# LDEO-CREW/Pythonic-DISORT

Measured on AMD Instinct MI355X. Metric: column-solves/sec (32 streams, 20 layers), higher is better.
Workload: dtype f64

## Files before the change

### pythonic-disort_amd/csrc/rtd_eig.hip

```cpp
#include <cstdlib>
#include <type_traits>

#include "rtd_device.h"

namespace {

#define RTD_FENCE() asm volatile("" ::: "memory")
#ifndef RTD_XOR_DPP
#define RTD_XOR_DPP 0x818E
#endif

constexpr __host__ __device__ int dpp_xor_ctrl(int mask) {
  return mask == 1 ? 0xB1 : mask == 2 ? 0x4E : mask == 3 ? 0x1B : mask == 7 ? 0x141 : mask == 8 ? 0x128 : mask == 15 ? 0x140 : -1;
}

template <int MASK>
__device__ __forceinline__ double xor_lane(double v) {
  if constexpr (MASK >= 32) return __shfl_xor(v, MASK, 64);
  int lo = __double2loint(v), hi = __double2hiint(v);
  constexpr int ctrl = dpp_xor_ctrl(MASK);
  if constexpr (ctrl >= 0 && ((RTD_XOR_DPP >> MASK) & 1)) {
    lo = __builtin_amdgcn_update_dpp(0, lo, ctrl, 0xF, 0xF, true);
    hi = __builtin_amdgcn_update_dpp(0, hi, ctrl, 0xF, 0xF, true);
  } else {
// ... 102 lines not shown
template <int B, int E, typename F>
__device__ __forceinline__ void static_for(F&& f) {
  if constexpr (B < E) {
    f(std::integral_constant<int, B>{});
    static_for<B + 1, E>(f);
  }
}

template <int NP, int K>
__device__ __forceinline__ double bcast_lane(double v) {
  if constexpr (NP == 16) {
    int lo = __double2loint(v), hi = __double2hiint(v);
    lo = __builtin_amdgcn_update_dpp(0, lo, 0x150 + K, 0xF, 0xF, true);
    hi = __builtin_amdgcn_update_dpp(0, hi, 0x150 + K, 0xF, 0xF, true);
    return __hiloint2double(hi, lo);
  } else if constexpr (NP == 64) {
    return __hiloint2double(__builtin_amdgcn_readlane(__double2hiint(v), K), __builtin_amdgcn_readlane(__double2loint(v), K));
  } else {
    return __shfl(v, K, NP);
  }
}

template <int NP, int K, int I, bool ORDERED = false>
struct CholRowDpp {
  static __device__ __forceinline__ void run(double (&col)[NP], const double f) {
    if constexpr (ORDERED) {
      if constexpr (I == K + 1 || I == NP - 1)
        asm volatile("v_fmac_f64_dpp %0, -%0, %1 row_newbcast:%2 row_mask:0xf bank_mask:0xf\n\ts_nop 1" : "+v"(col[I]) : "v"(f), "n"(K % 16));
      else
        asm volatile("v_fmac_f64_dpp %0, -%0, %1 row_newbcast:%2 row_mask:0xf bank_mask:0xf" : "+v"(col[I]) : "v"(f), "n"(K % 16));
    } else {
      if constexpr (I == K + 1 || I == NP - 1)
        asm("v_fmac_f64_dpp %0, -%0, %1 row_newbcast:%2 row_mask:0xf bank_mask:0xf\n\ts_nop 1" : "+v"(col[I]) : "v"(f), "n"(K % 16));
      else
        asm("v_fmac_f64_dpp %0, -%0, %1 row_newbcast:%2 row_mask:0xf bank_mask:0xf" : "+v"(col[I]) : "v"(f), "n"(K % 16));
    }
    CholRowDpp<NP, K, I + 1, ORDERED>::run(col, f);
  }
};
template <int NP, int K, bool ORDERED>
struct CholRowDpp<NP, K, NP, ORDERED> {
  static __device__ __forceinline__ void run(double (&)[NP], const double) {}
};

template <int NP, int K>
struct CholStep {
  static __device__ __forceinline__ void run(double (&col)[NP], double& diag, const int j) {
    const double akk = bcast_lane<NP, K>(col[K]);
    const double f = (j > K) ? col[K] * fast_rcp(akk) : 0.0;
    diag = (j == K) ? akk : diag;
    if constexpr (RTD_CHOL_FMAC_DPP && NP == 16) {
      CholRowDpp<NP, K, K + 1>::run(col, f);
    } else {
#pragma unroll
      for (int i = K + 1; i < NP; ++i) col[i] = fma(-bcast_lane<NP, K>(col[i]), f, col[i]);
    }
    CholStep<NP, K + 1>::run(col, diag, j);
  }
};
template <int NP>
struct CholStep<NP, NP> {
  static __device__ __forceinline__ void run(double (&)[NP], double&, const int) {}
};
template <int I>
struct RowFmacDpp {
  static __device__ __forceinline__ void run(double (&acc)[32], const double y0, const double y1, const double coef) {
    asm("v_fmac_f64_dpp %0, %1, %2 row_newbcast:%3 row_mask:0xf bank_mask:0xf" : "+v"(acc[I]) : "v"(y0), "v"(coef), "n"(I));
    asm("v_fmac_f64_dpp %0, %1, %2 row_newbcast:%3 row_mask:0xf bank_mask:0xf" : "+v"(acc[16 + I]) : "v"(y1), "v"(coef), "n"(I));
    if constexpr (I + 1 < 16) RowFmacDpp<I + 1>::run(acc, y0, y1, coef);
  }
};

template <int I>
struct RowFmacDpp64 {
  static __device__ __forceinline__ void run(double (&acc)[64], const double (&y)[4], const double coef) {
    asm("v_fmac_f64_dpp %0, %1, %2 row_newbcast:%3 row_mask:0xf bank_mask:0xf" : "+v"(acc[I]) : "v"(y[0]), "v"(coef), "n"(I));
    asm("v_fmac_f64_dpp %0, %1, %2 row_newbcast:%3 row_mask:0xf bank_mask:0xf" : "+v"(acc[16 + I]) : "v"(y[1]), "v"(coef), "n"(I));
    asm("v_fmac_f64_dpp %0, %1, %2 row_newbcast:%3 row_mask:0xf bank_mask:0xf" : "+v"(acc[32 + I]) : "v"(y[2]), "v"(coef), "n"(I));
    asm("v_fmac_f64_dpp %0, %1, %2 row_newbcast:%3 row_mask:0xf bank_mask:0xf" : "+v"(acc[48 + I]) : "v"(y[3]), "v"(coef), "n"(I));
    if constexpr (I + 1 < 16) RowFmacDpp64<I + 1>::run(acc, y, coef);
  }
};

template <int K>
__device__ __forceinline__ void fmac_bcast(double& acc, const double src, const double mul) {
  asm("v_fmac_f64_dpp %0, %1, %2 row_newbcast:%3 row_mask:0xf bank_mask:0xf" : "+v"(acc) : "v"(src), "v"(mul), "n"(K));
}

template <int NP>
struct LRowN {
  double g[NP / 16];
  template <int R, bool PACKED>
  static __device__ __forceinline__ LRowN load(const double* L_, const int t) {
    constexpr int off = PACKED ? R * (R + 1) / 2 : R * (NP + 1);
    LRowN x;
#pragma unroll
    for (int gi = 0; gi < NP / 16; ++gi) x.g[gi] = 16 * gi <= R ? L_[off + 16 * gi + t] : 0.0;
    return x;
  }
};
template <int NP, int I, int IEND>
struct AxpyRowN {
  static __device__ __forceinline__ void run(double (&acc)[NP], const LRowN<NP>& row, const double mul) {
    if constexpr (I < IEND) {
      fmac_bcast<I % 16>(acc[I], row.g[I / 16], mul);
      AxpyRowN<NP, I + 1, IEND>::run(acc, row, mul);
    }
  }
};
template <int NP, int I, int IEND>
struct DotRowN {
  static __device__ __forceinline__ void run(double (&a)[NP / 16], const LRowN<NP>& row, const double (&v)[NP]) {
    if constexpr (I < IEND) {
      fmac_bcast<I % 16>(a[I / 16], row.g[I / 16], v[I]);
      DotRowN<NP, I + 1, IEND>::run(a, row, v);
    }
  }
};

template <int NP>
__device__ __forceinline__ double transpose_reduce_scaled(const double (&a)[NP], const double s, const int j) {
  constexpr int O = NP / 2;
  const bool hi = (j & O) != 0;
  double v[O];
#pragma unroll
  for (int i = 0; i < O; ++i) v[i] = level_add<O, true>(a[i] * s, a[i + O] * s, hi);
  return transpose_reduce<O>(v, j);
}
template <int NP>
__device__ __forceinline__ double transpose_reduce_scaled2(const double (&a)[NP], const double s, const double (&b)[NP], const double t, const int j) {
  constexpr int O = NP / 2;
  const bool hi = (j & O) != 0;
  double v[O];
#pragma unroll
  for (int i = 0; i < O; ++i) v[i] = level_add<O, true>(fma(b[i], t, a[i] * s), fma(b[i + O], t, a[i + O] * s), hi);
  return transpose_reduce<O>(v, j);
}

template <int K>
__device__ __forceinline__ double row_bcast16(double v) {
  int lo = __double2loint(v), hi = __double2hiint(v);
  lo = __builtin_amdgcn_update_dpp(0, lo, 0x150 + K, 0xF, 0xF, true);
  hi = __builtin_amdgcn_update_dpp(0, hi, 0x150 + K, 0xF, 0xF, true);
  return __hiloint2double(hi, lo);
}
template <int K, int KEND>
struct CholPanel32 {
  static __device__ __forceinline__ void run(double (&col)[32], double& diag, double& dmine, const int row, const int jj) {
    constexpr int PR = K / 16, KL = K % 16;
    const double akk = row_bcast16<KL>(col[K]);
    const double r = fast_rcp(akk);
    const bool mine = row == PR;
    const double f = (mine && jj > KL) ? col[K] * r : 0.0;
    diag = (mine && jj == KL) ? akk : diag;
    dmine = (mine && jj == KL) ? r : dmine;
    CholRowDpp<32, K, K + 1, true>::run(col, f);
    if constexpr (K + 1 < KEND) CholPanel32<K + 1, KEND>::run(col, diag, dmine, row, jj);
  }
};
__device__ __forceinline__ double cholesky_columns32(double (&col)[32], const int j, double* scratch) {
  typedef double v4d __attribute__((ext_vector_type(4)));
  const int lane = threadIdx.x, g = lane >> 5, row = (lane >> 4) & 1, jj = lane & 15;
  double diag = 1.0, dmine = 0.0;
  CholPanel32<0, 16>::run(col, diag, dmine, row, jj);
  double* sX = scratch;
  double* sXd = scratch + 512;
  __syncthreads();
  if (row == 0) {
#pragma unroll
    for (int i = 0; i < 16; ++i) {
      sX[(g * 16 + jj) * 16 + i] = col[16 + i];
      sXd[(g * 16 + jj) * 16 + i] = col[16 + i] * dmine;
    }
  }
  __syncthreads();
  v4d acc[2];
#pragma unroll
  for (int pg = 0; pg < 2; ++pg) {
    acc[pg] = v4d{0.0, 0.0, 0.0, 0.0};
#pragma unroll
    for (int t = 0; t < 4; ++t) {
      const int e = (pg * 16 + 4 * t + (lane >> 4)) * 16 + (lane & 15);
      acc[pg] = __builtin_amdgcn_mfma_f64_16x16x4f64(sXd[e], sX[e], acc[pg], 0, 0, 0);
    }
  }
  __syncthreads();
  double* sS = scratch;
#pragma unroll
  for (int pg = 0; pg < 2; ++pg)
#pragma unroll
    for (int q = 0; q < 4; ++q) sS[(pg * 16 + 4 * q + (lane >> 4)) * 16 + (lane & 15)] = acc[pg][q];
  __syncthreads();
  if (row == 1) {
#pragma unroll
    for (int i = 0; i < 16; ++i) col[16 + i] -= sS[(g * 16 + i) * 16 + jj];
  }
  CholPanel32<16, 32>::run(col, diag, dmine, row, jj);
  const double rinv = fast_rsqrt(diag);
#pragma unroll
  for (int i = 0; i < 32; ++i) col[i] = (i >= j) ? col[i] * rinv : 0.0;
  __syncthreads();
  return rinv;
}

template <int NP>
__device__ __forceinline__ double cholesky_columns(double (&col)[NP], const int j) {
  double diag = 1.0;
  CholStep<NP, 0>::run(col, diag, j);
  const double rinv = fast_rsqrt(diag);
#pragma unroll
  for (int i = 0; i < NP; ++i) col[i] = (i >= j) ? col[i] * rinv : 0.0;
  return rinv;
}

struct ProbId {
  long pid;
  int c, m, l;
  int mg;
  bool valid;
// ... 140 lines not shown
    const double delta = ay - ax;
    const double g2 = 2.0 * gamma;
    const float df = (float)delta, gf = (float)g2;
    const float r2f = fmaf(df, df, fmaf(gf, gf, 1e-36f));
    const float rhof = r2f * __builtin_amdgcn_rsqf(r2f);
    const float denf = df + copysignf(rhof, df);
    const double tt = (double)(gf * __builtin_amdgcn_rcpf(denf));
    const double t2 = fma(tt, tt, 1.0);
    const double c = fast_rsqrt(t2);
    const double cinv = t2 * c;
    notconv |= (gamma * gamma > RTD_JAC_TOL * ax * ay) ? 1 : 0;
    const double nax = fma(-tt, gamma, ax), nay = fma(tt, gamma, ay);
    const double a = -tt * (sy * rx), b = tt * (sx * ry);
    const double nsx = c * sx, nsy = c * sy, nrx = cinv * rx, nry = cinv * ry;
    if constexpr (SW == 0) {
#pragma unroll
      for (int i = 0; i < H; ++i) {
        const double xi = xh[i], yi = yh[i];
        xh[i] = fma(a, yi, xi);
        yh[i] = xor_lane<MK>(fma(b, xi, yi));
      }
      ax = nax;
      ay = xor_lane<MK>(nay);
      sx = nsx;
      rx = nrx;
      sy = xor_lane<MK>(nsy);
      ry = xor_lane<MK>(nry);
    } else {
      const bool swp = (p & SW) != 0;
      const double pxx = swp ? b : 1.0, pxy = swp ? 1.0 : a, pyx = swp ? 1.0 : b, pyy = swp ? a : 1.0;
#pragma unroll
      for (int i = 0; i < H; ++i) {
        const double xi = xh[i], yi = yh[i];
        xh[i] = fma(pxy, yi, pxx * xi);
        yh[i] = xor_lane<MK>(fma(pyy, yi, pyx * xi));
      }
      ax = swp ? nay : nax;
      ay = xor_lane<MK>(swp ? nax : nay);
      sx = swp ? nsy : nsx;
      rx = swp ? nry : nrx;
      sy = xor_lane<MK>(swp ? nsx : nsy);
      ry = xor_lane<MK>(swp ? nrx : nry);
      const int t = swp ? iy : ix;
      iy = swp ? ix : iy;
      ix = t;
    }
    iy = xor_lane_i<MK>(iy);
    FastPairStep<NP, S + 1>::run(xh, yh, ax, ay, ix, iy, p, notconv, sx, sy, rx, ry);
  }
};
template <int NP>
struct FastPairStep<NP, NP - 1> {
  static __device__ __forceinline__ void run(double (&)[NP / 2], double (&)[NP / 2], double&, double&, int&, int&, const int, int&,
                                             double&, double&, double&, double&) {}
};

__host__ __device__ constexpr int tri(int r, int c) { return r * (r + 1) / 2 + c; }

#ifdef RTD_EIG_STAMPS
#define RTD_ESTAMP(k)                                      \
  {                                                        \
    __builtin_amdgcn_sched_barrier(0);                     \
    est[k] = (long long)__builtin_amdgcn_s_memtime();      \
    __builtin_amdgcn_sched_barrier(0);                     \
  }
#else
#define RTD_ESTAMP(k)
#endif

template <int NP, int JV>
__global__ __launch_bounds__(64, (NP <= 16 ? RTD_EIGEN_WAVES : NP == 32 ? RTD_EIGEN32_WAVES : 1)) void rtd_eigen_kernel(RtdDev d) {
  constexpr int GPW = 64 / NP;
  constexpr bool PACKED = NP == 32;
  constexpr int LD = NP + 1;
  constexpr int LSIZE = PACKED ? NP * (NP + 1) / 2 : NP * LD;
  __shared__ double sL[GPW][LSIZE];
  auto lix = [](const int r, const int c) { return PACKED ? tri(r, c) : r * LD + c; };
  __shared__ double sV[GPW][4][NP];
  constexpr int TROWS = NP == 32 ? 32 : 1;
  __shared__ double sTab[NP == 32 ? TROWS * NP : 1];
  __shared__ double sCoef[NP == 32 ? GPW * TROWS : 1];
  __shared__ double sY0[NP == 32 ? TROWS : 1];
  double w[NP];
  double xe_sum = 0.0, xo_sum = 0.0;
#ifdef RTD_EIG_STAMPS
  long long est[12];
  for (int k = 0; k < 12; ++k) est[k] = 0;
  int est_sweeps = 0;
#endif
  RTD_ESTAMP(0);
  double mu0_c = 1.0, I0_c = 0.0;
  if (d.beam) {
    const int c0 = locate<NP>(d).c;
    mu0_c = d.mu0[c0];
    I0_c = d.I0[c0];
  }
  {
  const int grp = threadIdx.x / NP, j = threadIdx.x % NP;
  const ProbId id = locate<NP>(d);
  const int P = d.P, m = id.m, c = id.c, l = id.l;
  double* L_ = sL[grp];
  double* dinv = sV[grp][3];
  const double* wl = d.wleg + ((long)c * d.L + l) * P;
  const double om = d.omega[(long)c * d.L + l];
  const double* Ym = d.Y + (long)m * P * NP;

  const double invmu_j = d.invmu[j], S_j = d.S[j];
  if constexpr (JV == 3 && NP == 16) {
    typedef double v4d __attribute__((ext_vector_type(4)));
    typedef unsigned int u2 __attribute__((ext_vector_type(2)));
    const int tx = threadIdx.x, i16 = tx & 15, k4 = tx >> 4;
    int chunk = (int)((long)blockIdx.x % (d.nsel > 0 ? d.nsel : (d.ln + GPW - 1) / GPW));
    if (d.nsel > 0) chunk = d.chunk_sel[(long)c * d.nsel + chunk];
    if (chunk < 0) chunk = (d.ln + GPW - 1) / GPW;
    double cm_ = 0.0;
    for (int ell = id.mg + j; ell < P; ell += NP) cm_ = fmax(cm_, fabs(0.5 * om * wl[ell]));
    const unsigned long long livemask = __ballot(cm_ > 1e-8);
    if (d.beam && ((livemask >> (NP * grp)) & 0xffffull)) {
      const double* Y0b = d.Y0 + ((long)c * d.M + m) * P;
      for (int ell = id.mg; ell < P; ell += 2) {
        xe_sum = fma(om * wl[ell] * Ym[(long)ell * NP + j], Y0b[ell], xe_sum);
        if (ell + 1 < P) xo_sum = fma(om * wl[ell + 1] * Ym[(long)(ell + 1) * NP + j], Y0b[ell + 1], xo_sum);
      }
    }
    const double S_i = d.S[i16], invmu_c = d.invmu[i16];
    v4d accP[GPW], accQ[GPW];
#pragma unroll
    for (int g = 0; g < GPW; ++g)
#pragma unroll
      for (int q = 0; q < 4; ++q) accP[g][q] = accQ[g][q] = (4 * q + k4 == i16) ? invmu_c : 0.0;
    const double* wlg[GPW];
    double omg[GPW];
#pragma unroll
    for (int g = 0; g < GPW; ++g) {
      const int slot = chunk * GPW + g;
      const int sl = slot < d.ln ? slot : d.ln - 1;
      const int lg = d.ln == d.L ? d.lperm[(long)c * d.L + sl] : d.l0 + sl;
      wlg[g] = d.wleg + ((long)c * d.L + lg) * P;
      omg[g] = ((livemask >> (NP * g)) & 0xffffull) ? -d.omega[(long)c * d.L + lg] : 0.0;
    }
    for (int base = id.mg; base < P; base += 8) {
      const int le = base + 2 * k4, lo = le + 1;
      const double ye = le < P ? Ym[(long)le * NP + i16] * S_i : 0.0;
      const double yo = lo < P ? Ym[(long)lo * NP + i16] * S_i : 0.0;
#pragma unroll
      for (int g = 0; g < GPW; ++g) {
        const double ce = le < P ? omg[g] * wlg[g][le] : 0.0, co = lo < P ? omg[g] * wlg[g][lo] : 0.0;
        accP[g] = __builtin_amdgcn_mfma_f64_16x16x4f64(ce * ye, ye, accP[g], 0, 0, 0);
        accQ[g] = __builtin_amdgcn_mfma_f64_16x16x4f64(co * yo, yo, accQ[g], 0, 0, 0);
      }
    }
    double pcol[NP], qcol[NP];
    auto transpose4 = [](const v4d (&acc)[GPW], const int q, double (&out)[NP]) {
      unsigned r[4][2];
#pragma unroll
      for (int g = 0; g < 4; ++g) {
        r[g][0] = (unsigned)__double2loint(acc[g][q]);
        r[g][1] = (unsigned)__double2hiint(acc[g][q]);
      }
#pragma unroll
      for (int h = 0; h < 2; ++h) {
        const u2 s01 = __builtin_amdgcn_permlane16_swap(r[0][h], r[1][h], false, false);
        const u2 s23 = __builtin_amdgcn_permlane16_swap(r[2][h], r[3][h], false, false);
        const u2 t02 = __builtin_amdgcn_permlane32_swap(s01[0], s23[0], false, false);
        const u2 t13 = __builtin_amdgcn_permlane32_swap(s01[1], s23[1], false, false);
        r[0][h] = t02[0];
        r[2][h] = t02[1];
        r[1][h] = t13[0];
        r[3][h] = t13[1];
      }
#pragma unroll
      for (int k = 0; k < 4; ++k) out[4 * q + k] = __hiloint2double((int)r[k][1], (int)r[k][0]);
    };
    if constexpr (GPW == 4) {
#pragma unroll
      for (int q = 0; q < 4; ++q) {
        transpose4(accP, q, pcol);
        transpose4(accQ, q, qcol);
      }
    }
    dinv[j] = cholesky_columns<NP>(pcol, j);
    cholesky_columns<NP>(qcol, j);
#pragma unroll
    for (int i = 0; i < NP; ++i)
        if (!PACKED || j <= i) L_[lix(i, 0) + j] = pcol[i];
    __syncthreads();
#pragma unroll
    for (int i = 0; i < NP; ++i) {
      double a = 0.0;
#pragma unroll
      for (int r = i; r < NP; ++r) a += L_[lix(r, i)] * qcol[r];
      w[i] = a;
    }
  } else if constexpr (NP == 32) {
    const int le = id.mg + 2 * j, lo = le + 1;
    const double wle = le < P ? wl[le] : 0.0, wlo = lo < P ? wl[lo] : 0.0;
    const double* Y0b = d.Y0 + ((long)c * d.M + m) * P;
    const double y0e = (d.beam && le < P) ? Y0b[le] : 0.0, y0o = (d.beam && lo < P) ? Y0b[lo] : 0.0;
    double cmax = fmax(fabs(0.5 * om * wle), fabs(0.5 * om * wlo));
    cmax = fmax(cmax, xor_lane<1>(cmax));
    cmax = fmax(cmax, xor_lane<2>(cmax));
    cmax = fmax(cmax, xor_lane<4>(cmax));
    cmax = fmax(cmax, xor_lane<8>(cmax));
    cmax = fmax(cmax, xor_lane<16>(cmax));
    const double live = (cmax > 1e-8) ? 1.0 : 0.0;
    auto assemble = [&](const int first, const double wmine, const double y0mine, double (&col)[NP], double& beam_sum) {
      const int nrows = (P - first + 1) / 2;
      __syncthreads();
      {
        constexpr int TRIPS = TROWS * (NP / 2) / 64;
        double2 v[TRIPS];
#pragma unroll
        for (int t = 0; t < TRIPS; ++t) {
          const int idx = t * 64 + (int)threadIdx.x, row = idx / (NP / 2), q = idx % (NP / 2);
          const int ell = first + 2 * row < P ? first + 2 * row : P - 1;
          v[t] = *reinterpret_cast<const double2*>(Ym + (long)ell * NP + 2 * q);
        }
#pragma unroll
        for (int t = 0; t < TRIPS; ++t) {
          const int idx = t * 64 + (int)threadIdx.x;
          if (idx < nrows * (NP / 2)) *reinterpret_cast<double2*>(&sTab[idx * 2]) = v[t];
        }
      }
      sCoef[grp * TROWS + j] = om * wmine;
      if (grp == 0) sY0[j] = y0mine;
      __syncthreads();
      double acc[NP];
#pragma unroll
      for (int i = 0; i < NP; ++i) acc[i] = 0.0;
      const int jj = j & 15;
      for (int k = 0; k < nrows; ++k) {
        const double y0 = sTab[k * NP + jj], y1 = sTab[k * NP + 16 + jj];
        const double coef = sCoef[grp * TROWS + k] * (j < 16 ? y0 : y1);
        beam_sum = fma(live * coef, sY0[k], beam_sum);
        RowFmacDpp<0>::run(acc, y0, y1, coef);
      }
#pragma unroll
      for (int i = 0; i < NP; ++i) col[i] = (i == j ? invmu_j : 0.0) - d.S[i] * (live * acc[i]) * S_j;
    };
    {
      double pcol[NP];
      assemble(id.mg, wle, y0e, pcol, xe_sum);
      RTD_ESTAMP(1);
      dinv[j] = cholesky_columns32(pcol, j, sTab);
      RTD_ESTAMP(2);
#pragma unroll
      for (int i = 0; i < NP; ++i)
        if (!PACKED || j <= i) L_[lix(i, 0) + j] = pcol[i];
    }
    double qcol[NP];
    assemble(id.mg + 1, wlo, y0o, qcol, xo_sum);
    RTD_ESTAMP(3);
    cholesky_columns32(qcol, j, sTab);
    RTD_ESTAMP(4);
    __syncthreads();
    {
      const int t16 = j & 15;
#pragma unroll
      for (int i = 0; i < NP; ++i) w[i] = 0.0;
      static_for<0, NP>([&](auto rc) {
        constexpr int r = decltype(rc)::value;
        const LRowN<NP> row = LRowN<NP>::template load<r, PACKED>(L_, t16);
        AxpyRowN<NP, 0, r + 1>::run(w, row, qcol[r]);
        if constexpr ((r & 3) == 3) RTD_FENCE();
      });
    }
  } else if constexpr (NP == 64) {
    typedef const double __attribute__((address_space(4))) kdouble;
    kdouble* wk = (kdouble*)wl;
    kdouble* Y0k = (kdouble*)(d.Y0 + ((long)c * d.M + m) * P);
    const int jj = j & 15;
    const bool jr1 = (j & 16) != 0, jr2 = (j & 32) != 0;
    double cmax = 0.0;
    {
      const int l0 = id.mg + j, l1 = l0 + NP;
      if (l0 < P) cmax = fabs(0.5 * om * wl[l0]);
      if (l1 < P) cmax = fmax(cmax, fabs(0.5 * om * wl[l1]));
      cmax = fmax(cmax, xor_lane<1>(cmax));
      cmax = fmax(cmax, xor_lane<2>(cmax));
      cmax = fmax(cmax, xor_lane<4>(cmax));
      cmax = fmax(cmax, xor_lane<8>(cmax));
      cmax = fmax(cmax, xor_lane<16>(cmax));
      cmax = fmax(cmax, xor_lane<32>(cmax));
    }
    const double live = (cmax > 1e-8) ? 1.0 : 0.0;
    auto assemble = [&](const int first, double (&col)[NP], double& beam_sum) {
      double acc[NP];
#pragma unroll
      for (int i = 0; i < NP; ++i) acc[i] = 0.0;
      constexpr int CH = 8;
      double yv[CH][4], yn[CH][4], wv[CH], wn[CH], y0v[CH], y0n[CH];
#pragma unroll
      for (int e = 0; e < CH; ++e) {
        const int ell = first + 2 * e < P ? first + 2 * e : P - 1;
#pragma unroll
        for (int g = 0; g < 4; ++g) yv[e][g] = Ym[(long)ell * NP + 16 * g + jj];
        wv[e] = wk[ell];
        y0v[e] = Y0k[ell];
      }
#pragma unroll 1
      for (int base = first; base < P; base += 2 * CH) {
#pragma unroll
        for (int e = 0; e < CH; ++e) {
          const int ell = base + 2 * (CH + e) < P ? base + 2 * (CH + e) : P - 1;
#pragma unroll
          for (int g = 0; g < 4; ++g) yn[e][g] = Ym[(long)ell * NP + 16 * g + jj];
          wn[e] = wk[ell];
          y0n[e] = Y0k[ell];
        }
#pragma unroll
        for (int e = 0; e < CH; ++e) {
          if (base + 2 * e < P) {
            const double ylo = jr1 ? yv[e][1] : yv[e][0], yhi = jr1 ? yv[e][3] : yv[e][2];
            const double coef = om * wv[e] * (jr2 ? yhi : ylo);
            beam_sum = fma(coef, y0v[e], beam_sum);
            RowFmacDpp64<0>::run(acc, yv[e], coef);
          }
        }
#pragma unroll
        for (int e = 0; e < CH; ++e) {
#pragma unroll
          for (int g = 0; g < 4; ++g) yv[e][g] = yn[e][g];
          wv[e] = wn[e];
          y0v[e] = y0n[e];
        }
      }
      beam_sum *= live;
#pragma unroll
      for (int i = 0; i < NP; ++i) col[i] = (i == j ? invmu_j : 0.0) - d.S[i] * (live * acc[i]) * S_j;
    };
    {
      double pcol[NP];
      assemble(id.mg, pcol, xe_sum);
      RTD_ESTAMP(1);
      dinv[j] = cholesky_columns<NP>(pcol, j);
      RTD_ESTAMP(2);
#pragma unroll
      for (int i = 0; i < NP; ++i) L_[lix(i, 0) + j] = pcol[i];
    }
    double qcol[NP];
    assemble(id.mg + 1, qcol, xo_sum);
    RTD_ESTAMP(3);
    cholesky_columns<NP>(qcol, j);
    RTD_ESTAMP(4);
    __syncthreads();
    {
      const int t16 = j & 15;
#pragma unroll
      for (int i = 0; i < NP; ++i) w[i] = 0.0;
      static_for<0, NP>([&](auto rc) {
        constexpr int r = decltype(rc)::value;
        const LRowN<NP> row = LRowN<NP>::template load<r, PACKED>(L_, t16);
        AxpyRowN<NP, 0, r + 1>::run(w, row, qcol[r]);
        if constexpr ((r & 3) == 3) RTD_FENCE();
      });
    }
  } else {
  double acc_e[NP], acc_o[NP];
#pragma unroll
  for (int i = 0; i < NP; ++i) acc_e[i] = acc_o[i] = 0.0;
  double cmax = 0.0;
  const double* Y0b = d.Y0 + ((long)c * d.M + m) * P;
  for (int ell = id.mg; ell < P; ell += 2) {
    {
      const double cl = 0.5 * om * wl[ell];
      cmax = fmax(cmax, fabs(cl));
      const double* Yr = Ym + (long)ell * NP;
      const double coef = 2.0 * cl * Yr[j];
      if (d.beam) xe_sum = fma(coef, Y0b[ell], xe_sum);
#pragma unroll
      for (int i = 0; i < NP; ++i) acc_e[i] += coef * Yr[i];
    }
    if (ell + 1 < P) {
      const double cl = 0.5 * om * wl[ell + 1];
      cmax = fmax(cmax, fabs(cl));
      const double* Yr = Ym + (long)(ell + 1) * NP;
      const double coef = 2.0 * cl * Yr[j];
      if (d.beam) xo_sum = fma(coef, Y0b[ell + 1], xo_sum);
#pragma unroll
      for (int i = 0; i < NP; ++i) acc_o[i] += coef * Yr[i];
    }
  }
  if (!(cmax > 1e-8)) {
#pragma unroll
    for (int i = 0; i < NP; ++i) acc_e[i] = acc_o[i] = 0.0;
    xe_sum = xo_sum = 0.0;
  }
  {
    double pcol[NP], qcol[NP];
#pragma unroll
    for (int i = 0; i < NP; ++i) {
      const double Si = d.S[i];
      pcol[i] = (i == j ? invmu_j : 0.0) - Si * acc_e[i] * S_j;
      qcol[i] = (i == j ? invmu_j : 0.0) - Si * acc_o[i] * S_j;
    }
    RTD_ESTAMP(1);
    dinv[j] = cholesky_columns<NP>(pcol, j);
    RTD_ESTAMP(2);
    RTD_ESTAMP(3);
    cholesky_columns<NP>(qcol, j);
    RTD_ESTAMP(4);
#pragma unroll
    for (int i = 0; i < NP; ++i)
        if (!PACKED || j <= i) L_[lix(i, 0) + j] = pcol[i];
    __syncthreads();
#pragma unroll
    for (int i = 0; i < NP; ++i) {
      double a = 0.0;
#pragma unroll
      for (int r = i; r < NP; ++r) a += L_[lix(r, i)] * qcol[r];
      w[i] = a;
    }
  }
  }
  RTD_ESTAMP(5);
  int nsweep = 0;
  bool converged = false;
  {
    constexpr int H = NP / 2;
    const int u = j / H, p = j % H;
    double xh[H], yh[H];
#pragma unroll
    for (int i = 0; i < H; ++i) {
      const double recv = xor_lane<H>(u ? w[i] : w[H + i]);
      xh[i] = u ? recv : w[i];
      yh[i] = u ? w[H + i] : recv;
    }
    int ix = p, iy = p + H;
    for (int sweep = 0; sweep < 40; ++sweep) {
      int notconv = 0;
      double ax = 0.0, ay = 0.0;
#pragma unroll
      for (int i = 0; i < H; ++i) {
        ax = fma(xh[i], xh[i], ax);
        ay = fma(yh[i], yh[i], ay);
      }
      ax += xor_lane<H>(ax);
      ay += xor_lane<H>(ay);
      if constexpr (RTD_JAC_FAST && NP >= 32) {
        double sx = 1.0, sy = 1.0, rx = 1.0, ry = 1.0;
        FastPairStep<NP, 0>::run(xh, yh, ax, ay, ix, iy, p, notconv, sx, sy, rx, ry);
#pragma unroll
        for (int i = 0; i < H; ++i) {
          xh[i] *= sx;
          yh[i] *= sy;
        }
      } else {
        PairStep<NP, 0>::run(xh, yh, ax, ay, ix, iy, p, notconv);
      }
      ++nsweep;
      if (!__any(notconv)) {
        converged = true;
        break;
      }
    }
#pragma unroll
    for (int i = 0; i < H; ++i) {
      const double recv = xor_lane<H>(u ? xh[i] : yh[i]);
      w[i] = u ? recv : xh[i];
      w[H + i] = u ? yh[i] : recv;
    }
    int* where = reinterpret_cast<int*>(sV[grp][0]);
    where[u ? iy : ix] = j;
    __syncthreads();
    const int src = where[j];
#pragma unroll
    for (int i = 0; i < NP; ++i) w[i] = __shfl(w[i], src, NP);
    __syncthreads();
  }
  RTD_ESTAMP(6);
#ifdef RTD_EIG_STAMPS
  est_sweeps = nsweep;
#endif
  if (threadIdx.x == 0 && nsweep > *(volatile int*)d.sweeps) atomicMax(d.sweeps, nsweep);
  if (!converged && threadIdx.x == 0) rtd_raise(d, RTD_ST_JACOBI, id.mg, id.c);
  }
  int tx = threadIdx.x;
  asm volatile("" : "+v"(tx));
  const int grp = tx / NP, j = tx % NP;
  const ProbId id = locate<NP>(d, tx);
  const int P = d.P, m = id.m, c = id.c, l = id.l;
  const bool valid = id.valid;
  const long base = id.pid;
  double* L_ = sL[grp];
  double* v0 = sV[grp][0];
  double* v1 = sV[grp][1];
  double* v2 = sV[grp][2];
  double* dinv = sV[grp][3];
  const double* wl = d.wleg + ((long)c * d.L + l) * P;
  const double om = d.omega[(long)c * d.L + l];
  const double* Ym = d.Y + (long)m * P * NP;
  double invmu_j = d.invmu[j], T_j = d.T[j];
  double dts;
  {
    const double* ts0 = d.taus0 + (long)c * (d.L + 1);
    dts = ts0[l + 1] - ts0[l];
  }
  double k2 = 0.0;
#pragma unroll
  for (int i = 0; i < NP; ++i) k2 += w[i] * w[i];
  const double rk0 = fast_rsqrt(k2), kj = k2 * rk0;
  if (valid && !(k2 > 0.0 && k2 < 1e300)) rtd_raise(d, RTD_ST_CHOL, id.mg, id.c);
  double zc[NP];
  {
#pragma unroll
    for (int i = 0; i < NP; ++i) zc[i] = w[i] * rk0;
  }

  double ya[NP];
  if constexpr (NP >= 32) {
    const int t16 = j & 15;
#pragma unroll
    for (int i = 0; i < NP; ++i) ya[i] = zc[i];
    static_for<0, NP>([&](auto kc) {
      constexpr int r = NP - 1 - decltype(kc)::value;
      ya[r] *= dinv[r];
      if constexpr (r > 0) {
        const LRowN<NP> row = LRowN<NP>::template load<r, PACKED>(L_, t16);
        AxpyRowN<NP, 0, r>::run(ya, row, -ya[r]);
      }
      if constexpr ((r & 3) == 0) RTD_FENCE();
    });
  } else {
#pragma unroll
  for (int i = NP - 1; i >= 0; --i) {
    double a = zc[i];
#pragma unroll
    for (int r = i + 1; r < NP; ++r) a -= L_[lix(r, i)] * ya[r];
    ya[i] = a * dinv[i];
    RTD_FENCE();
  }
  }
  RTD_ESTAMP(7);
  double ekj = 0.0;
  if constexpr (NP == 32) ekj = exp(-kj * dts);
  asm volatile("" : "+v"(invmu_j), "+v"(T_j), "+v"(dts));
  auto store_Y = [&]() {
    if constexpr (NP == 32) {
      asm volatile("" : "+v"(ya[0]), "+v"(ya[1]), "+v"(ya[2]), "+v"(ya[3]), "+v"(ya[4]), "+v"(ya[5]), "+v"(ya[6]), "+v"(ya[7]), "+v"(ya[8]),
                        "+v"(ya[9]), "+v"(ya[10]), "+v"(ya[11]), "+v"(ya[12]), "+v"(ya[13]), "+v"(ya[14]), "+v"(ya[15]));
      asm volatile("" : "+v"(ya[16]), "+v"(ya[17]), "+v"(ya[18]), "+v"(ya[19]), "+v"(ya[20]), "+v"(ya[21]), "+v"(ya[22]), "+v"(ya[23]),
                        "+v"(ya[24]), "+v"(ya[25]), "+v"(ya[26]), "+v"(ya[27]), "+v"(ya[28]), "+v"(ya[29]), "+v"(ya[30]), "+v"(ya[31]));
    }
    if (valid) {
      double* Ym = d.Ym + base * NP * NP;
#pragma unroll
      for (int i = 0; i < NP; ++i) Ym[i * NP + j] = ya[i];
      d.kk[base * NP + j] = kj;
      if constexpr (NP != 32) ekj = exp(-kj * dts);
      d.Ek[base * NP + j] = ekj;
    }
  };
  if constexpr (NP != 32) store_Y();

  double bv_up = 0.0, bv_dn = 0.0;
  if (d.beam) {
    const double mu0 = mu0_c;
    const double fac = I0_c * (0.25 / M_PI) * (id.mg == 0 ? 1.0 : 2.0);
    const double xe = fac * xe_sum, xo = fac * xo_sum;
    const double txd = 2.0 * T_j * xe * invmu_j;
    v0[j] = txd;
    __syncthreads();
    double qv;
    {
      double tq = 0.0;
#pragma unroll
      for (int i = 0; i < NP; ++i) tq += ya[i] * v0[i];
      tq *= k2;
      if constexpr (NP == 32) {
        qv = transpose_reduce_scaled<NP>(ya, tq, j);
      } else {
        double x[NP];
#pragma unroll
        for (int i = 0; i < NP; ++i) x[i] = ya[i] * tq;
        qv = transpose_reduce<NP>(x, j);
      }
    }
    const double rmu0 = fast_rcp(mu0);
    const double rhat = 2.0 * T_j * xo * invmu_j * rmu0 - qv;
    v1[j] = rhat;
    __syncthreads();
    double g = 0.0;
#pragma unroll
    for (int r = 0; r < NP; ++r) g += ((!PACKED || r >= j) ? L_[lix(r, 0) + j] : 0.0) * v1[r];
    v2[j] = g;
    __syncthreads();
    double h = 0.0;
#pragma unroll
    for (int i = 0; i < NP; ++i) h += zc[i] * v2[i];
    h *= fast_rcp(rmu0 * rmu0 - k2);
    double sh, e;
    if constexpr (NP == 32) {
      sh = transpose_reduce_scaled<NP>(ya, h, j);
      e = transpose_reduce_scaled<NP>(zc, h, j);
    } else {
      double x[NP];
#pragma unroll
      for (int i = 0; i < NP; ++i) x[i] = ya[i] * h;
      sh = transpose_reduce<NP>(x, j);
#pragma unroll
      for (int i = 0; i < NP; ++i) x[i] = zc[i] * h;
      e = transpose_reduce<NP>(x, j);
    }
    __syncthreads();
    v2[j] = e;
    __syncthreads();
    double ps = 0.0;
#pragma unroll
    for (int r = 0; r < NP; ++r) ps += ((!PACKED || r <= j) ? L_[lix(j, 0) + r] : 0.0) * v2[r];
    const double rT = fast_rcp(T_j);
    const double s_j = sh * rT;
    const double d_j = mu0 * (txd - ps) * rT;
    bv_up = 0.5 * (s_j + d_j);
    bv_dn = 0.5 * (s_j - d_j);
    if constexpr (NP != 32) {
      if (valid) {
        d.Bv[base * 2 * NP + j] = bv_up;
        d.Bv[base * 2 * NP + NP + j] = bv_dn;
      }
    }
    if (valid && !(fabs(s_j) + fabs(d_j) < 1e300)) rtd_raise(d, RTD_ST_BEAM, id.mg, id.c);
  }
  __syncthreads();
  RTD_ESTAMP(8);
  double aa[NP];
  if constexpr (NP == 32) {
    store_Y();
    const int t16 = j & 15;
    static_for<0, NP>([&](auto rc) {
      constexpr int r = decltype(rc)::value;
      const LRowN<NP> row = LRowN<NP>::template load<r, PACKED>(L_, t16);
      double a[NP / 16] = {};
      DotRowN<NP, 0, r + 1>::run(a, row, zc);
      aa[r] = r >= 16 ? a[0] + a[1] : a[0];
      if constexpr ((r & 3) == 3) RTD_FENCE();
    });
    asm volatile("" : "+v"(aa[0]), "+v"(aa[1]), "+v"(aa[2]), "+v"(aa[3]), "+v"(aa[4]), "+v"(aa[5]), "+v"(aa[6]), "+v"(aa[7]), "+v"(aa[8]),
                      "+v"(aa[9]), "+v"(aa[10]), "+v"(aa[11]), "+v"(aa[12]), "+v"(aa[13]), "+v"(aa[14]), "+v"(aa[15]));
    asm volatile("" : "+v"(aa[16]), "+v"(aa[17]), "+v"(aa[18]), "+v"(aa[19]), "+v"(aa[20]), "+v"(aa[21]), "+v"(aa[22]), "+v"(aa[23]),
                      "+v"(aa[24]), "+v"(aa[25]), "+v"(aa[26]), "+v"(aa[27]), "+v"(aa[28]), "+v"(aa[29]), "+v"(aa[30]), "+v"(aa[31]));
  } else if constexpr (NP == 64) {
    const int t16 = j & 15;
    static_for<0, NP>([&](auto rc) {
      constexpr int r = decltype(rc)::value;
      const LRowN<NP> row = LRowN<NP>::template load<r, PACKED>(L_, t16);
      double a[NP / 16] = {};
      DotRowN<NP, 0, r + 1>::run(a, row, zc);
      aa[r] = (a[0] + a[1]) + (a[2] + a[3]);
      if constexpr ((r & 3) == 3) RTD_FENCE();
    });
  } else {
#pragma unroll
  for (int i = 0; i < NP; ++i) {
    double a = 0.0;
#pragma unroll
    for (int r = 0; r <= i; ++r) a += L_[lix(i, r)] * zc[r];
    aa[i] = a;
    if (NP != 64 || (i & 7) == 7) RTD_FENCE();
  }
  }
  if (valid) {
    double* Am = d.Am + base * NP * NP;
#pragma unroll
    for (int i = 0; i < NP; ++i) Am[i * NP + j] = aa[i];
    if constexpr (NP == 32) {
      if (d.beam) {
        d.Bv[base * 2 * NP + j] = bv_up;
        d.Bv[base * 2 * NP + NP + j] = bv_dn;
      }
    }
  }

  if (d.Ns > 0 && id.mg == 0) {
    const bool act = true;
    double yl[NP == 32 ? NP : 1], al[NP == 32 ? NP : 1];
    if constexpr (NP == 32) {
      const double* Yg = d.Ym + base * NP * NP;
      const double* Ag = d.Am + base * NP * NP;
#pragma unroll
      for (int i = 0; i < NP; ++i) {
        yl[i] = Yg[i * NP + j];
        al[i] = Ag[i * NP + j];
      }
    }
    const auto& ya_t = [&]() -> const double(&)[NP] { if constexpr (NP == 32) return yl; else return ya; }();
    const auto& aa_t = [&]() -> const double(&)[NP] { if constexpr (NP == 32) return al; else return aa; }();
    double zn = 0.0;
#pragma unroll
    for (int i = 0; i < NP; ++i) zn += ya_t[i] * (d.T[i] * d.invmu[i]);
    zn *= -0.5 * kj;
    if (valid && act) d.zneg[((long)c * d.L + l) * NP + j] = zn;
    const double* sp = d.spoly + ((long)c * d.L + l) * d.Ns;
    const double rk = rk0;
    const double ts_top = 0.0, ts_bot = d.taus0[(long)c * (d.L + 1) + l + 1] - d.taus0[(long)c * (d.L + 1) + l];
    double vtu = 0.0, vtd = 0.0, vbu = 0.0, vbd = 0.0, tpt = 1.0, tpb = 1.0;
    for (int q = 0; q < d.Ns; ++q) {
      double bneg = 0.0, bpos = 0.0, ratio = 1.0, pw_pos = rk, pw_neg = -rk;
      for (int jj = q; jj < d.Ns; ++jj) {
        bpos += ratio * sp[jj] * pw_pos;
        bneg += ratio * sp[jj] * pw_neg;
        ratio *= (double)(jj + 1);
        pw_pos *= rk;
        pw_neg *= -rk;
      }
      const double a = zn * bneg, b = -zn * bpos;
      const double sab = a + b, dab = (a - b) * rk;
      const double rT = 1.0 / T_j;
      double up, dn;
      if constexpr (NP == 32) {
        up = transpose_reduce_scaled2<NP>(ya_t, sab, aa_t, -dab, j) * rT;
        dn = transpose_reduce_scaled2<NP>(ya_t, sab, aa_t, dab, j) * rT;
      } else {
        double xu[NP], xd[NP];
#pragma unroll
        for (int i = 0; i < NP; ++i) {
          const double py = ya_t[i] * sab, pa = aa_t[i] * dab;
          xu[i] = py - pa;
          xd[i] = py + pa;
        }
        up = transpose_reduce<NP>(xu, j) * rT;
        dn = transpose_reduce<NP>(xd, j) * rT;
      }
      if (valid && act) {
        double* dq = d.dq + (((long)c * d.L + l) * d.Ns + q) * 2 * NP;
        dq[j] = up;
        dq[NP + j] = dn;
      }
      vtu += up * tpt;
      vtd += dn * tpt;
      vbu += up * tpb;
      vbd += dn * tpb;
      tpt *= ts_top;
      tpb *= ts_bot;
    }
    if (valid && act) {
      double* vb = d.vb + ((long)c * d.L + l) * 4 * NP;
      vb[j] = vtu;
      vb[NP + j] = vtd;
      vb[2 * NP + j] = vbu;
      vb[3 * NP + j] = vbd;
    }
    __syncthreads();
  }
  RTD_ESTAMP(9);
#ifdef RTD_EIG_STAMPS
  if (threadIdx.x == 0 && blockIdx.x % 4099 == 7)
    printf("EIGSTAMP np %d m %d sweeps %d : asmP %lld cholP %lld asmQ %lld cholQ %lld F %lld jacobi %lld order+Y %lld beam %lld A+thermal %lld total %lld\n",
           NP, id.mg, est_sweeps, est[1] - est[0], est[2] - est[1], est[3] - est[2], est[4] - est[3], est[5] - est[4], est[6] - est[5],
           est[7] - est[6], est[8] - est[7], est[9] - est[8], est[9] - est[0]);
#endif

}

__device__ __forceinline__ void ybar_column(int m, int P, double x, double* out, long stride) {
  double v = 1.0;
  const double sx = sqrt(fmax(0.0, 1.0 - x * x));
  for (int jj = 1; jj <= m; ++jj) v *= sqrt((2.0 * jj - 1.0) / (2.0 * jj)) * sx;
  for (int ell = 0; ell < m && ell < P; ++ell) out[ell * stride] = 0.0;
  if (m >= P) return;
  double ym1 = 0.0, y = v;
  out[m * stride] = y;
  for (int ell = m; ell + 1 < P; ++ell) {
    const double yn = ((2.0 * ell + 1.0) * x * y - sqrt((double)(ell + m) * (double)(ell - m)) * ym1) /
                      sqrt((double)(ell + 1 - m) * (double)(ell + 1 + m));
    ym1 = y;
    y = yn;
    out[(ell + 1) * stride] = y;
  }
}

__global__ void rtd_tables_quad_kernel(RtdDev d) {
  const int t = blockIdx.x * blockDim.x + threadIdx.x;
  if (t >= d.M * d.NP) return;
  const int m = t / d.NP, i = t % d.NP;
// ... 63 lines not shown
```

Baseline: 238,500.

## Use DPP broadcast products and skip eigenvector shuffle for NP=16 eigen kernel

For the 16-stream case, the L^T q product, the forward substitution and the A product now use DPP row-broadcast FMAs instead of LDS-indexed scalar loops. The beam-source solve replaces shared-memory vector exchanges and barriers with in-register dot_bcast16 chains. The column permutation after the eigen sort is no longer done with LDS writes, barriers and shuffles; each lane keeps its destination column and writes outputs there. This removes several __syncthreads and LDS round trips, at the cost of more register pressure and inline asm that must respect DPP hazards (an explicit s_nop is added for this).

```diff
diff --git a/pythonic-disort_amd/csrc/rtd_eig.hip b/pythonic-disort_amd/csrc/rtd_eig.hip
--- a/pythonic-disort_amd/csrc/rtd_eig.hip
+++ b/pythonic-disort_amd/csrc/rtd_eig.hip
@@ -208,9 +208,37 @@
   }
 };
 
-template <int K>
+template <int K, bool NEG = false>
 __device__ __forceinline__ void fmac_bcast(double& acc, const double src, const double mul) {
-  asm("v_fmac_f64_dpp %0, %1, %2 row_newbcast:%3 row_mask:0xf bank_mask:0xf" : "+v"(acc) : "v"(src), "v"(mul), "n"(K));
+  if constexpr (NEG)
+    asm("v_fmac_f64_dpp %0, %1, -%2 row_newbcast:%3 row_mask:0xf bank_mask:0xf" : "+v"(acc) : "v"(src), "v"(mul), "n"(K));
+  else
+    asm("v_fmac_f64_dpp %0, %1, %2 row_newbcast:%3 row_mask:0xf bank_mask:0xf" : "+v"(acc) : "v"(src), "v"(mul), "n"(K));
+}
+
+__device__ __forceinline__ double dot_bcast16(const double src, const double (&m)[16]) {
+  double acc = 0.0;
+  asm("s_nop 1\n\t"
+      "v_fmac_f64_dpp %0, %1, %2 row_newbcast:0 row_mask:0xf bank_mask:0xf\n\t"
+      "v_fmac_f64_dpp %0, %1, %3 row_newbcast:1 row_mask:0xf bank_mask:0xf\n\t"
+      "v_fmac_f64_dpp %0, %1, %4 row_newbcast:2 row_mask:0xf bank_mask:0xf\n\t"
+      "v_fmac_f64_dpp %0, %1, %5 row_newbcast:3 row_mask:0xf bank_mask:0xf\n\t"
+      "v_fmac_f64_dpp %0, %1, %6 row_newbcast:4 row_mask:0xf bank_mask:0xf\n\t"
+      "v_fmac_f64_dpp %0, %1, %7 row_newbcast:5 row_mask:0xf bank_mask:0xf\n\t"
+      "v_fmac_f64_dpp %0, %1, %8 row_newbcast:6 row_mask:0xf bank_mask:0xf\n\t"
+      "v_fmac_f64_dpp %0, %1, %9 row_newbcast:7 row_mask:0xf bank_mask:0xf\n\t"
+      "v_fmac_f64_dpp %0, %1, %10 row_newbcast:8 row_mask:0xf bank_mask:0xf\n\t"
+      "v_fmac_f64_dpp %0, %1, %11 row_newbcast:9 row_mask:0xf bank_mask:0xf\n\t"
+      "v_fmac_f64_dpp %0, %1, %12 row_newbcast:10 row_mask:0xf bank_mask:0xf\n\t"
+      "v_fmac_f64_dpp %0, %1, %13 row_newbcast:11 row_mask:0xf bank_mask:0xf\n\t"
+      "v_fmac_f64_dpp %0, %1, %14 row_newbcast:12 row_mask:0xf bank_mask:0xf\n\t"
+      "v_fmac_f64_dpp %0, %1, %15 row_newbcast:13 row_mask:0xf bank_mask:0xf\n\t"
+      "v_fmac_f64_dpp %0, %1, %16 row_newbcast:14 row_mask:0xf bank_mask:0xf\n\t"
+      "v_fmac_f64_dpp %0, %1, %17 row_newbcast:15 row_mask:0xf bank_mask:0xf"
+      : "+v"(acc)
+      : "v"(src), "v"(m[0]), "v"(m[1]), "v"(m[2]), "v"(m[3]), "v"(m[4]), "v"(m[5]), "v"(m[6]), "v"(m[7]), "v"(m[8]), "v"(m[9]),
+        "v"(m[10]), "v"(m[11]), "v"(m[12]), "v"(m[13]), "v"(m[14]), "v"(m[15]));
+  return acc;
 }
 
 template <int NP>
@@ -225,12 +253,12 @@
     return x;
   }
 };
-template <int NP, int I, int IEND>
+template <int NP, int I, int IEND, bool NEG = false>
 struct AxpyRowN {
   static __device__ __forceinline__ void run(double (&acc)[NP], const LRowN<NP>& row, const double mul) {
     if constexpr (I < IEND) {
-      fmac_bcast<I % 16>(acc[I], row.g[I / 16], mul);
-      AxpyRowN<NP, I + 1, IEND>::run(acc, row, mul);
+      fmac_bcast<I % 16, NEG>(acc[I], row.g[I / 16], mul);
+      AxpyRowN<NP, I + 1, IEND, NEG>::run(acc, row, mul);
     }
   }
 };
@@ -261,6 +289,18 @@
 #pragma unroll
   for (int i = 0; i < O; ++i) v[i] = level_add<O, true>(fma(b[i], t, a[i] * s), fma(b[i + O], t, a[i + O] * s), hi);
   return transpose_reduce<O>(v, j);
+}
+
+template <int NP, bool PACKED>
+__device__ __forceinline__ void lt_product(double (&w)[NP], const double* L_, const double (&q)[NP], const int t16) {
+#pragma unroll
+  for (int i = 0; i < NP; ++i) w[i] = 0.0;
+  static_for<0, NP>([&](auto rc) {
+    constexpr int r = decltype(rc)::value;
+    const LRowN<NP> row = LRowN<NP>::template load<r, PACKED>(L_, t16);
+    AxpyRowN<NP, 0, r + 1>::run(w, row, q[r]);
+    if constexpr ((r & 3) == 3) RTD_FENCE();
+  });
 }
 
 template <int K>
@@ -567,6 +607,7 @@
   __shared__ double sCoef[NP == 32 ? GPW * TROWS : 1];
   __shared__ double sY0[NP == 32 ? TROWS : 1];
   double w[NP];
+  int ecol = 0;
   double xe_sum = 0.0, xo_sum = 0.0;
 #ifdef RTD_EIG_STAMPS
   long long est[12];
@@ -670,13 +711,7 @@
     for (int i = 0; i < NP; ++i)
         if (!PACKED || j <= i) L_[lix(i, 0) + j] = pcol[i];
     __syncthreads();
-#pragma unroll
-    for (int i = 0; i < NP; ++i) {
-      double a = 0.0;
-#pragma unroll
-      for (int r = i; r < NP; ++r) a += L_[lix(r, i)] * qcol[r];
-      w[i] = a;
-    }
+    lt_product<NP, PACKED>(w, L_, qcol, j & 15);
   } else if constexpr (NP == 32) {
     const int le = id.mg + 2 * j, lo = le + 1;
     const double wle = le < P ? wl[le] : 0.0, wlo = lo < P ? wl[lo] : 0.0;
@@ -739,17 +774,7 @@
     cholesky_columns32(qcol, j, sTab);
     RTD_ESTAMP(4);
     __syncthreads();
-    {
-      const int t16 = j & 15;
-#pragma unroll
-      for (int i = 0; i < NP; ++i) w[i] = 0.0;
-      static_for<0, NP>([&](auto rc) {
-        constexpr int r = decltype(rc)::value;
-        const LRowN<NP> row = LRowN<NP>::template load<r, PACKED>(L_, t16);
-        AxpyRowN<NP, 0, r + 1>::run(w, row, qcol[r]);
-        if constexpr ((r & 3) == 3) RTD_FENCE();
-      });
-    }
+    lt_product<NP, PACKED>(w, L_, qcol, j & 15);
   } else if constexpr (NP == 64) {
     typedef const double __attribute__((address_space(4))) kdouble;
     kdouble* wk = (kdouble*)wl;
@@ -829,17 +854,7 @@
     cholesky_columns<NP>(qcol, j);
     RTD_ESTAMP(4);
     __syncthreads();
-    {
-      const int t16 = j & 15;
-#pragma unroll
-      for (int i = 0; i < NP; ++i) w[i] = 0.0;
-      static_for<0, NP>([&](auto rc) {
-        constexpr int r = decltype(rc)::value;
-        const LRowN<NP> row = LRowN<NP>::template load<r, PACKED>(L_, t16);
-        AxpyRowN<NP, 0, r + 1>::run(w, row, qcol[r]);
-        if constexpr ((r & 3) == 3) RTD_FENCE();
-      });
-    }
+    lt_product<NP, PACKED>(w, L_, qcol, j & 15);
   } else {
   double acc_e[NP], acc_o[NP];
 #pragma unroll
@@ -889,12 +904,16 @@
     for (int i = 0; i < NP; ++i)
         if (!PACKED || j <= i) L_[lix(i, 0) + j] = pcol[i];
     __syncthreads();
-#pragma unroll
-    for (int i = 0; i < NP; ++i) {
-      double a = 0.0;
-#pragma unroll
-      for (int r = i; r < NP; ++r) a += L_[lix(r, i)] * qcol[r];
-      w[i] = a;
+    if constexpr (NP == 16) {
+      lt_product<NP, PACKED>(w, L_, qcol, j);
+    } else {
+#pragma unroll
+      for (int i = 0; i < NP; ++i) {
+        double a = 0.0;
+#pragma unroll
+        for (int r = i; r < NP; ++r) a += L_[lix(r, i)] * qcol[r];
+        w[i] = a;
+      }
     }
   }
   }
@@ -945,13 +964,17 @@
       w[i] = u ? recv : xh[i];
       w[H + i] = u ? yh[i] : recv;
     }
-    int* where = reinterpret_cast<int*>(sV[grp][0]);
-    where[u ? iy : ix] = j;
-    __syncthreads();
-    const int src = where[j];
-#pragma unroll
-    for (int i = 0; i < NP; ++i) w[i] = __shfl(w[i], src, NP);
-    __syncthreads();
+    if constexpr (NP == 16) {
+      ecol = u ? iy : ix;
+    } else {
+      int* where = reinterpret_cast<int*>(sV[grp][0]);
+      where[u ? iy : ix] = j;
+      __syncthreads();
+      const int src = where[j];
+#pragma unroll
+      for (int i = 0; i < NP; ++i) w[i] = __shfl(w[i], src, NP);
+      __syncthreads();
+    }
   }
   RTD_ESTAMP(6);
 #ifdef RTD_EIG_STAMPS
@@ -963,6 +986,7 @@
   int tx = threadIdx.x;
   asm volatile("" : "+v"(tx));
   const int grp = tx / NP, j = tx % NP;
+  const int je = NP == 16 ? ecol : j;
   const ProbId id = locate<NP>(d, tx);
   const int P = d.P, m = id.m, c = id.c, l = id.l;
   const bool valid = id.valid;
@@ -993,7 +1017,7 @@
   }
 
   double ya[NP];
-  if constexpr (NP >= 32) {
+  if constexpr (NP >= 16) {
     const int t16 = j & 15;
 #pragma unroll
     for (int i = 0; i < NP; ++i) ya[i] = zc[i];
@@ -1002,7 +1026,7 @@
       ya[r] *= dinv[r];
       if constexpr (r > 0) {
         const LRowN<NP> row = LRowN<NP>::template load<r, PACKED>(L_, t16);
-        AxpyRowN<NP, 0, r>::run(ya, row, -ya[r]);
+        AxpyRowN<NP, 0, r, NP <= 32>::run(ya, row, NP <= 32 ? ya[r] : -ya[r]);
       }
       if constexpr ((r & 3) == 0) RTD_FENCE();
     });
@@ -1030,10 +1054,10 @@
     if (valid) {
       double* Ym = d.Ym + base * NP * NP;
 #pragma unroll
-      for (int i = 0; i < NP; ++i) Ym[i * NP + j] = ya[i];
-      d.kk[base * NP + j] = kj;
+      for (int i = 0; i < NP; ++i) Ym[i * NP + je] = ya[i];
+      d.kk[base * NP + je] = kj;
       if constexpr (NP != 32) ekj = exp(-kj * dts);
-      d.Ek[base * NP + j] = ekj;
+      d.Ek[base * NP + je] = ekj;
     }
   };
   if constexpr (NP != 32) store_Y();
@@ -1044,55 +1068,79 @@
     const double fac = I0_c * (0.25 / M_PI) * (id.mg == 0 ? 1.0 : 2.0);
     const double xe = fac * xe_sum, xo = fac * xo_sum;
     const double txd = 2.0 * T_j * xe * invmu_j;
-    v0[j] = txd;
-    __syncthreads();
-    double qv;
-    {
-      double tq = 0.0;
-#pragma unroll
-      for (int i = 0; i < NP; ++i) tq += ya[i] * v0[i];
-      tq *= k2;
+    double sh, ps;
+    if constexpr (NP == 16) {
+      double x[NP];
+      const double tq = dot_bcast16(txd, ya) * k2;
+#pragma unroll
+      for (int i = 0; i < NP; ++i) x[i] = ya[i] * tq;
+      const double qv = transpose_reduce<NP>(x, j);
+      const double rmu0 = fast_rcp(mu0);
+      const double rhat = 2.0 * T_j * xo * invmu_j * rmu0 - qv;
+      double lc[NP];
+#pragma unroll
+      for (int r = 0; r < NP; ++r) lc[r] = L_[lix(r, 0) + j];
+      const double g = dot_bcast16(rhat, lc);
+      const double h = dot_bcast16(g, zc) * fast_rcp(rmu0 * rmu0 - k2);
+#pragma unroll
+      for (int i = 0; i < NP; ++i) x[i] = ya[i] * h;
+      sh = transpose_reduce<NP>(x, j);
+      const double e = dot_bcast16(sh, lc);
+      double lr[NP];
+#pragma unroll
+      for (int r = 0; r < NP; ++r) lr[r] = L_[lix(j, 0) + r];
+      ps = dot_bcast16(e, lr);
+    } else {
+      v0[j] = txd;
+      __syncthreads();
+      double qv;
+      {
+        double tq = 0.0;
+#pragma unroll
+        for (int i = 0; i < NP; ++i) tq += ya[i] * v0[i];
+        tq *= k2;
+        if constexpr (NP == 32) {
+          qv = transpose_reduce_scaled<NP>(ya, tq, j);
+        } else {
+          double x[NP];
+#pragma unroll
+          for (int i = 0; i < NP; ++i) x[i] = ya[i] * tq;
+          qv = transpose_reduce<NP>(x, j);
+        }
+      }
+      const double rmu0 = fast_rcp(mu0);
+      const double rhat = 2.0 * T_j * xo * invmu_j * rmu0 - qv;
+      v1[j] = rhat;
+      __syncthreads();
+      double g = 0.0;
+#pragma unroll
+      for (int r = 0; r < NP; ++r) g += ((!PACKED || r >= j) ? L_[lix(r, 0) + j] : 0.0) * v1[r];
+      v2[j] = g;
+      __syncthreads();
+      double h = 0.0;
+#pragma unroll
+      for (int i = 0; i < NP; ++i) h += zc[i] * v2[i];
+      h *= fast_rcp(rmu0 * rmu0 - k2);
+      double e;
       if constexpr (NP == 32) {
-        qv = transpose_reduce_scaled<NP>(ya, tq, j);
+        sh = transpose_reduce_scaled<NP>(ya, h, j);
+        e = transpose_reduce_scaled<NP>(zc, h, j);
       } else {
         double x[NP];
 #pragma unroll
-        for (int i = 0; i < NP; ++i) x[i] = ya[i] * tq;
-        qv = transpose_reduce<NP>(x, j);
-      }
-    }
-    const double rmu0 = fast_rcp(mu0);
-    const double rhat = 2.0 * T_j * xo * invmu_j * rmu0 - qv;
-    v1[j] = rhat;
-    __syncthreads();
-    double g = 0.0;
-#pragma unroll
-    for (int r = 0; r < NP; ++r) g += ((!PACKED || r >= j) ? L_[lix(r, 0) + j] : 0.0) * v1[r];
-    v2[j] = g;
-    __syncthreads();
-    double h = 0.0;
-#pragma unroll
-    for (int i = 0; i < NP; ++i) h += zc[i] * v2[i];
-    h *= fast_rcp(rmu0 * rmu0 - k2);
-    double sh, e;
-    if constexpr (NP == 32) {
-      sh = transpose_reduce_scaled<NP>(ya, h, j);
-      e = transpose_reduce_scaled<NP>(zc, h, j);
-    } else {
-      double x[NP];
-#pragma unroll
-      for (int i = 0; i < NP; ++i) x[i] = ya[i] * h;
-      sh = transpose_reduce<NP>(x, j);
-#pragma unroll
-      for (int i = 0; i < NP; ++i) x[i] = zc[i] * h;
-      e = transpose_reduce<NP>(x, j);
-    }
-    __syncthreads();
-    v2[j] = e;
-    __syncthreads();
-    double ps = 0.0;
-#pragma unroll
-    for (int r = 0; r < NP; ++r) ps += ((!PACKED || r <= j) ? L_[lix(j, 0) + r] : 0.0) * v2[r];
+        for (int i = 0; i < NP; ++i) x[i] = ya[i] * h;
+        sh = transpose_reduce<NP>(x, j);
+#pragma unroll
+        for (int i = 0; i < NP; ++i) x[i] = zc[i] * h;
+        e = transpose_reduce<NP>(x, j);
+      }
+      __syncthreads();
+      v2[j] = e;
+      __syncthreads();
+      ps = 0.0;
+#pragma unroll
+      for (int r = 0; r < NP; ++r) ps += ((!PACKED || r <= j) ? L_[lix(j, 0) + r] : 0.0) * v2[r];
+    }
     const double rT = fast_rcp(T_j);
     const double s_j = sh * rT;
     const double d_j = mu0 * (txd - ps) * rT;
@@ -1124,14 +1172,15 @@
                       "+v"(aa[9]), "+v"(aa[10]), "+v"(aa[11]), "+v"(aa[12]), "+v"(aa[13]), "+v"(aa[14]), "+v"(aa[15]));
     asm volatile("" : "+v"(aa[16]), "+v"(aa[17]), "+v"(aa[18]), "+v"(aa[19]), "+v"(aa[20]), "+v"(aa[21]), "+v"(aa[22]), "+v"(aa[23]),
                       "+v"(aa[24]), "+v"(aa[25]), "+v"(aa[26]), "+v"(aa[27]), "+v"(aa[28]), "+v"(aa[29]), "+v"(aa[30]), "+v"(aa[31]));
-  } else if constexpr (NP == 64) {
+  } else if constexpr (NP == 16 || NP == 64) {
     const int t16 = j & 15;
     static_for<0, NP>([&](auto rc) {
       constexpr int r = decltype(rc)::value;
       const LRowN<NP> row = LRowN<NP>::template load<r, PACKED>(L_, t16);
       double a[NP / 16] = {};
       DotRowN<NP, 0, r + 1>::run(a, row, zc);
-      aa[r] = (a[0] + a[1]) + (a[2] + a[3]);
+      if constexpr (NP == 16) aa[r] = a[0];
+      else aa[r] = (a[0] + a[1]) + (a[2] + a[3]);
       if constexpr ((r & 3) == 3) RTD_FENCE();
     });
   } else {
@@ -1147,7 +1196,7 @@
   if (valid) {
     double* Am = d.Am + base * NP * NP;
 #pragma unroll
-    for (int i = 0; i < NP; ++i) Am[i * NP + j] = aa[i];
+    for (int i = 0; i < NP; ++i) Am[i * NP + je] = aa[i];
     if constexpr (NP == 32) {
       if (d.beam) {
         d.Bv[base * 2 * NP + j] = bv_up;
@@ -1174,7 +1223,7 @@
 #pragma unroll
     for (int i = 0; i < NP; ++i) zn += ya_t[i] * (d.T[i] * d.invmu[i]);
     zn *= -0.5 * kj;
-    if (valid && act) d.zneg[((long)c * d.L + l) * NP + j] = zn;
+    if (valid && act) d.zneg[((long)c * d.L + l) * NP + je] = zn;
     const double* sp = d.spoly + ((long)c * d.L + l) * d.Ns;
     const double rk = rk0;
     const double ts_top = 0.0, ts_bot = d.taus0[(long)c * (d.L + 1) + l + 1] - d.taus0[(long)c * (d.L + 1) + l];
```

New measurement: 245,100, median of 6. 2.8% higher.
